# apple/ml-gmpi

Hardware: AMD Instinct MI355X
Metric: Mpix*planes/s (higher is better)
Workload: dtype f32; 1 GPU; FFHQ1024-shaped: 1024x1024, 96 planes, batch 4 views, bf16 storage; views_per_gpu=4, views_total=4, H=1024, W=1024, planes=96, variant=auto, strict_order=False, outputs=rgb+depth, parallelism=views sharded x1, poses=truncated-gaussian draw (seed 3) on every rank

## Files before the change

### include/gmpi_render.h

```cpp
#ifndef GMPI_RENDER_H
#define GMPI_RENDER_H

#include <stdint.h>

#ifdef __cplusplus
extern "C" {
#endif

#define GMPI_ABI_VERSION 2

enum { GMPI_DTYPE_F32 = 0, GMPI_DTYPE_BF16 = 1, GMPI_DTYPE_F16 = 2, GMPI_DTYPE_U8 = 3 };

enum {
    GMPI_FLAG_ALIGN_CORNERS = 1 << 0,
    GMPI_FLAG_OUT_PM1 = 1 << 1,
    GMPI_FLAG_CHECK_LAST_PLANE = 1 << 2,
    GMPI_FLAG_CHECK_RANGE = 1 << 3,
    GMPI_FLAG_STRICT_ORDER = 1 << 4,
    GMPI_FLAG_HINT_FRONTAL = 1 << 5,
    GMPI_FLAG_HINT_TILTED = 1 << 6,
    GMPI_FLAG_GRAD_OVERWRITE = 1 << 7,
    GMPI_FLAG_HINT_OBLIQUE = 1 << 8,
    GMPI_FLAG_ALL = (1 << 9) - 1
};

enum {
    GMPI_STATUS_OUT_OF_LAST_PLANE = 1u << 0,
    GMPI_STATUS_RGBA_RANGE = 1u << 1,
    GMPI_STATUS_CAMERA_BEHIND_PLANE = 1u << 2,
    GMPI_STATUS_BAD_VIEW_INDEX = 1u << 3
};
#define GMPI_STATUS_WORDS 4

enum {
    GMPI_VARIANT_AUTO = 0,
    GMPI_VARIANT_GATHER = 1,
    GMPI_VARIANT_LDS = 2,
    GMPI_VARIANT_WAVE = 3,
    GMPI_VARIANT_DMA = 4,
    GMPI_VARIANT_BAND = 5
};

enum {
    GMPI_OK = 0,
    GMPI_E_NULL = -1,
    GMPI_E_SHAPE = -2,
    GMPI_E_DTYPE = -3,
    GMPI_E_STRIDE = -4,
    GMPI_E_ABI = -5,
    GMPI_E_VARIANT = -6,
    GMPI_E_FLAGS = -7,
    GMPI_E_WORKSPACE = -8,
    GMPI_E_LAUNCH = -100
};

typedef struct GmpiRenderParams {
// ... 111 lines not shown
```

### ml-gmpi_amd/_lib.py

```python
import ctypes
import os
import subprocess

_PKG = os.path.dirname(os.path.abspath(__file__))
_SO = os.path.join(_PKG, "libgmpi_render.so")
_LIB = None

ABI_VERSION = 2
DTYPE_F32, DTYPE_BF16, DTYPE_F16 = 0, 1, 2
DTYPE_U8 = 3
FLAG_ALIGN_CORNERS, FLAG_OUT_PM1, FLAG_CHECK_LAST_PLANE, FLAG_CHECK_RANGE, FLAG_STRICT_ORDER, FLAG_HINT_FRONTAL, FLAG_HINT_TILTED = 1, 2, 4, 8, 16, 32, 64
FLAG_HINT_OBLIQUE = 256
FLAG_GRAD_OVERWRITE = 128
STATUS_OUT_OF_LAST_PLANE, STATUS_RGBA_RANGE, STATUS_CAMERA_BEHIND_PLANE, STATUS_BAD_VIEW_INDEX = 1, 2, 4, 8
STATUS_WORDS = 4
VARIANT_AUTO, VARIANT_GATHER, VARIANT_LDS, VARIANT_WAVE, VARIANT_DMA, VARIANT_BAND = 0, 1, 2, 3, 4, 5
VARIANTS = {"auto": VARIANT_AUTO, "gather": VARIANT_GATHER, "lds": VARIANT_LDS, "wave": VARIANT_WAVE, "band": VARIANT_BAND}

EXPORTS = (
    "gmpi_mpi_render_launch",
    "gmpi_render_workspace_bytes",
    "gmpi_render_backward_workspace_bytes",
    "gmpi_mpi_render_backward_launch",
    "gmpi_render_geometry_backward_workspace_bytes",
    "gmpi_mpi_render_geometry_backward_launch",
    "gmpi_mpi_render_backward_ex_launch",
    "gmpi_mpi_render_geometry_backward_ex_launch",
    "gmpi_mpi_render_shared_launch",
    "gmpi_mpi_render_shared_backward_launch",
    "gmpi_render_shared_supports",
    "gmpi_last_plane_uv_minmax_launch",
    "gmpi_rgba_range_check_launch",
    "gmpi_frames_to_uint8_launch",
    "gmpi_generate_rays_launch",
    "gmpi_alpha_depth_launch",
    "gmpi_light_blur_launch",
    "gmpi_light_shading_launch",
    "gmpi_light_apply_launch",
    "gmpi_light_apply_backward_launch",
    "gmpi_alpha_depth_backward_launch",
    "gmpi_alpha_depth_backward_ex_launch",
    "gmpi_selftest_division_launch",
    "gmpi_stream_probe_launch",
    "gmpi_query",
    "gmpi_version_string",
# ... 189 lines not shown
```

### ml-gmpi_amd/csrc/gmpi_abi.hip

```cpp
#include "gmpi_device.hpp"
#include "gmpi_shared.hpp"

#include "../../include/gmpi_render.h"

#include <atomic>
#include <cstdlib>

namespace gmpi {

hipError_t launch_gather(const KParams& p, int dtype, hipStream_t stream);
hipError_t launch_lds(const KParams& p, int dtype, int tune, hipStream_t stream);
hipError_t launch_backward(const KParams& p, int dtype, const float* g_rgb, const float* g_depth, const float* g_T, float* g_rgba,
                           const int64_t* gstride, bool tiles, hipStream_t stream);
bool lds_variant_supports(const KParams& p, int dtype);
int lds_variant_query(int what);
hipError_t launch_wave(const KParams& p, int dtype, int tune, hipStream_t stream);
bool wave_variant_supports(const KParams& p, int dtype);
hipError_t launch_band(const KParams& p, int dtype, int tune, hipStream_t stream);
bool band_variant_supports(const KParams& p, int dtype);
uint64_t band_workspace_bytes(const KParams& p, int dtype);
uint32_t* band_gate_words(const KParams& p, int dtype);
int band_pixels_wide(int dtype);
uint64_t backward_gather_workspace_bytes(const KParams& p);
uint64_t geometry_backward_workspace_bytes(const KParams& p, bool want_dhw);
hipError_t launch_shared(const KParams& p, int dtype, const SharedK& sh, hipStream_t stream);
hipError_t launch_shared_backward(const KParams& p, int dtype, const SharedK& sh, const SharedG& g, bool tiles, hipStream_t stream);
hipError_t launch_shared_forward(const KParams& p, int dtype, const SharedK& sh, hipStream_t stream);
bool shared_forward_supports(const KParams& p, int dtype, const SharedK& sh);
int shared_forward_query(int what);
hipError_t launch_u8(const KParams& p, hipStream_t stream);
bool u8_variant_supports(const KParams& p);
int u8_variant_query(int what);
hipError_t launch_backward_geometry(const KParams& p, int dtype, const float* g_rgb, const float* g_depth, const float* g_T, float* g_ray, float* g_eye,
                                    float* g_z, float* g_dhw, hipStream_t stream);

template <bool AC>
__global__ __launch_bounds__(256) void last_plane_uv_kernel(const KParams p, float* __restrict__ uv) {
    const int n = blockIdx.x;
    uint32_t bad_index = 0;
    const int m = view_mpi(p, n, bad_index);
    const float* dhw = p.dhw + (static_cast<int64_t>(m) * p.D + (p.D - 1)) * 3;
    const float d = dhw[0], ph = dhw[1], pw = dhw[2];
    const float ex = p.eye_pos[3 * n + 0], ey = p.eye_pos[3 * n + 1], ez = p.eye_pos[3 * n + 2];
    const float zdiff = d - ez;
    const int64_t HW = static_cast<int64_t>(p.H) * p.W;
    const float* rd = p.ray_dir + static_cast<int64_t>(n) * 3 * HW;
    const float inf = __builtin_inff();
    float mnu = inf, mxu = -inf, mnv = inf, mxv = -inf;
    bool nan = false;
    for (int64_t i = threadIdx.x; i < HW; i += blockDim.x) {
        float ix, iy, s, u, v;
        plane_coord<AC>(zdiff, ph, pw, ex, ey, rd[i], rd[HW + i], rd[2 * HW + i], 1.0f, 1.0f, ix, iy, s, u, v);
        nan |= (u != u) || (v != v);
        mnu = fminf(mnu, u), mxu = fmaxf(mxu, u), mnv = fminf(mnv, v), mxv = fmaxf(mxv, v);
    }
// ... 550 lines not shown
int gmpi_selftest_division_launch(uint64_t pairs, uint32_t seed, uint64_t* mismatches, void* stream) {
    if (mismatches == nullptr) return GMPI_E_NULL;
    if (pairs == 0) return GMPI_OK;
    const uint64_t want = (pairs + 255) / 256;
    const unsigned blocks = static_cast<unsigned>(want < 256u * 64u ? want : 256u * 64u);
    hipLaunchKernelGGL(selftest_division_kernel, dim3(blocks), dim3(256), 0, static_cast<hipStream_t>(stream), pairs, seed,
                       reinterpret_cast<unsigned long long*>(mismatches));
    return hip_rc(hipGetLastError());
}

int gmpi_stream_probe_launch(const void* buf, uint64_t bytes, uint32_t* sink, void* stream) {
    if (buf == nullptr) return GMPI_E_NULL;
    if (reinterpret_cast<uintptr_t>(buf) % 4 != 0) return GMPI_E_STRIDE;
    if (bytes < 4) return GMPI_OK;
    hipLaunchKernelGGL(stream_probe_kernel, dim3(256 * 2), dim3(256), 0, static_cast<hipStream_t>(stream), static_cast<const uint32_t*>(buf),
                       static_cast<int64_t>(bytes / 4), sink);
    return hip_rc(hipGetLastError());
}

int gmpi_query(int32_t what) {
    switch (what) {
        case 0: return GMPI_ABI_VERSION;
        case 1: return static_cast<int>(sizeof(GmpiRenderParams));
        case 2: return 950;
        case 3: case 4: case 5: return lds_variant_query(what);
        case 6: return 1;
        case 7: return 0;
        case 8: return 1;
        case 9: return static_cast<int>(kAutoBandMin);
        case 10: return static_cast<int>(kAutoBandMinF32);
        case 11: return 1;
        case 12: case 13: case 14: return shared_forward_query(what);
        case 16: case 17: case 18: case 20: return u8_variant_query(what);
        default: return -1;
    }
}

const char* gmpi_version_string(void) { return "ml-gmpi_amd 0.3 (gfx950, ABI 2)"; }

}
```

### ml-gmpi_amd/csrc/render_band.hip

```cpp
#include "gmpi_device.hpp"

#include <algorithm>
#include <cstdlib>
#include <type_traits>


namespace gmpi {
namespace band {

constexpr int kNT = 1024;
constexpr int SBW = 64, SBH = 8;
constexpr float kBoxEps = 1.0f / 64;
constexpr int kWindowCols16 = 2, kWindowCols32 = 2, kWindowCols32Deep = 2, kDeepPlanes = 128;
constexpr int kViewRotation = 1;
constexpr int kRunPieces = 2;
constexpr int kTicketTail = 16;
constexpr float kCoordLimit = 16384.0f;

typedef uint32_t u32x4 __attribute__((ext_vector_type(4)));
template <int V> using ic = std::integral_constant<int, V>;

template <int D0, int STEP>
__device__ __forceinline__ void dma16x2(uint32_t voff, uint32_t soff1, const u32x4& rsrc, uint32_t lds_dst, uint64_t m0, uint64_t m1);

#ifndef GMPI_BAND_PPT16
#define GMPI_BAND_PPT16 2
#endif
#ifndef GMPI_BAND_PPT32
#define GMPI_BAND_PPT32 2
#endif
template <typename TexT> struct Geo {
    static constexpr int kES = static_cast<int>(sizeof(TexT));
    static constexpr int NSB = kES == 2 ? 4 : 2;
    static constexpr int PPT = kES == 2 ? GMPI_BAND_PPT16 : GMPI_BAND_PPT32;
    static constexpr int WPS = SBH / PPT;
    static constexpr int kSubLanes = 64 * WPS;
    static constexpr int kThreads = NSB * kSubLanes;
    static constexpr int kWavesPerSimd = kThreads / 128;
    static_assert(kThreads <= kNT && SBH % PPT == 0, "waves");
    static constexpr int kTPI = 16 / kES;
    static constexpr int kCols = kES == 2 ? 10 : 20;
    static constexpr int kLineBytes = kCols * 16;
    static constexpr int kRowBytes = 4 * kLineBytes;
    static constexpr int kIPR = 4 * kCols;
    static constexpr int kMaxRows = 15;
    static constexpr int kCapItems = kMaxRows * kIPR;
    static constexpr int kSubBytes = kCapItems * 16;
    static constexpr int kBufBytes = NSB * kSubBytes;
    static constexpr int kRPP = kSubLanes / kIPR;
    static constexpr int kPassItems = kRPP * kIPR;
    static constexpr int kNP = (kMaxRows + kRPP - 1) / kRPP;
    static_assert(kNP == 3 || kNP == 5, "passes");
    static constexpr int kOffBytes = kThreads * 4;
    static constexpr int kLdsBytes = kOffBytes + 2 * kBufBytes;
};
static_assert(Geo<bf16_t>::kLdsBytes * 2 <= 160 * 1024 && Geo<f16_t>::kLdsBytes * 2 <= 160 * 1024 && Geo<float>::kLdsBytes * 2 <= 160 * 1024, "2 workgroups per CU");

__device__ __forceinline__ void dma16(uint32_t voff, uint32_t soff, const u32x4& rsrc, uint32_t lds_dst, uint64_t mask) {
    uint64_t save;
    asm volatile("s_mov_b64 %0, exec\n\ts_mov_b64 exec, %4\n\ts_mov_b32 m0, %3\n\ts_nop 0\n\tbuffer_load_dwordx4 %1, %2, %5 offen lds\n\ts_mov_b64 exec, %0"
                 : "=&s"(save) : "v"(voff), "s"(rsrc), "s"(lds_dst), "s"(mask), "s"(soff) : "memory");
}
template <int D0, int STEP>
__device__ __forceinline__ void dma16x3(uint32_t voff, uint32_t soff1, uint32_t soff2, const u32x4& rsrc, uint32_t lds_dst, uint64_t m0, uint64_t m1, uint64_t m2) {
    uint64_t save;
    asm volatile("s_mov_b64 %0, exec\n\t"
                 "s_mov_b64 exec, %4\n\ts_add_i32 m0, %3, %9\n\ts_nop 0\n\tbuffer_load_dwordx4 %1, %2, 0 offen lds\n\t"
                 "s_mov_b64 exec, %5\n\ts_add_i32 m0, %3, %10\n\ts_nop 0\n\tbuffer_load_dwordx4 %1, %2, %7 offen lds\n\t"
                 "s_mov_b64 exec, %6\n\ts_add_i32 m0, %3, %11\n\ts_nop 0\n\tbuffer_load_dwordx4 %1, %2, %8 offen lds\n\t"
                 "s_mov_b64 exec, %0"
                 : "=&s"(save) : "v"(voff), "s"(rsrc), "s"(lds_dst), "s"(m0), "s"(m1), "s"(m2), "s"(soff1), "s"(soff2), "i"(D0), "i"(D0 + STEP), "i"(D0 + 2 * STEP)
                 : "memory", "scc");
}
template <int D0, int STEP>
__device__ __forceinline__ void dma16x2(uint32_t voff, uint32_t soff1, const u32x4& rsrc, uint32_t lds_dst, uint64_t m0, uint64_t m1) {
    uint64_t save;
    asm volatile("s_mov_b64 %0, exec\n\t"
                 "s_mov_b64 exec, %4\n\ts_add_i32 m0, %3, %7\n\ts_nop 0\n\tbuffer_load_dwordx4 %1, %2, 0 offen lds\n\t"
                 "s_mov_b64 exec, %5\n\ts_add_i32 m0, %3, %8\n\ts_nop 0\n\tbuffer_load_dwordx4 %1, %2, %6 offen lds\n\t"
                 "s_mov_b64 exec, %0"
                 : "=&s"(save) : "v"(voff), "s"(rsrc), "s"(lds_dst), "s"(m0), "s"(m1), "s"(soff1), "i"(D0), "i"(D0 + STEP)
                 : "memory", "scc");
}
template <int D0, int STEP>
__device__ __forceinline__ void dma16x4(uint32_t voff, uint32_t s1, uint32_t s2, uint32_t s3, const u32x4& rsrc, uint32_t lds_dst, uint64_t m0, uint64_t m1, uint64_t m2, uint64_t m3) {
    uint64_t save;
    asm volatile("s_mov_b64 %0, exec\n\t"
                 "s_mov_b64 exec, %4\n\ts_add_i32 m0, %3, %11\n\ts_nop 0\n\tbuffer_load_dwordx4 %1, %2, 0 offen lds\n\t"
                 "s_mov_b64 exec, %5\n\ts_add_i32 m0, %3, %12\n\ts_nop 0\n\tbuffer_load_dwordx4 %1, %2, %8 offen lds\n\t"
// ... 178 lines not shown
            }
            __syncthreads();
            band_id = __builtin_amdgcn_readfirstlane(*word);
            __syncthreads();
        }
    }
#ifdef GMPI_TUNE
    if (p.flags & (1u << 19)) band_id = static_cast<int>(blockIdx.x % 8) * ((n_bands + 7) / 8) + static_cast<int>(blockIdx.x / 8);
#endif
    if (band_id >= n_bands) return;
    int n, brem;
    item_to_view(p, band_id, bands_x * bands_y, n, brem);
    if (view_gated_out(p, n)) return;
    int bxi, byi;
    band_pos(brem, bands_x, bands_y, p.band_cols, bxi, byi);
#ifdef GMPI_TUNE
    const bool stamp = (p.flags & (1u << 22)) != 0 && p.status != nullptr;
    uint64_t stamp_start = 0;
    if (stamp) asm volatile("s_memrealtime %0\n\ts_waitcnt lgkmcnt(0)" : "=s"(stamp_start));
#endif

    const int tid = threadIdx.x;
    auto fresh_tid = [&]() { int t = tid; asm volatile("" : "+v"(t)); return t; };
    const int wave = __builtin_amdgcn_readfirstlane(tid >> 6);
    const int sb = wave / WPS, wj = wave % WPS;
    const int lane = tid & 63;
    uint32_t bad_w = 0;
    View vw = view_setup<AC>(p, n, bad_w);
    vw.cx = cx, vw.cy = cy;
    const int D = p.D, H = p.H, W = p.W;
    const float* __restrict__ dhw = vw.dhw;
    const float ex = vw.ex, ey = vw.ey, ez = vw.ez;
    constexpr bool check_range = CHECK;
    const int64_t HW = vw.HW;
    const float* __restrict__ rdv = vw.rays;
    const TexT* __restrict__ vol = static_cast<const TexT*>(p.rgba) + static_cast<int64_t>(vw.m) * p.s_mpi;
    const int64_t s_chan = p.s_chan, s_row = p.s_row;

    check_camera_behind(p, vw, brem == 0 && tid == 0);

    const int px = bxi * (NSB * SBW) + sb * SBW + lane;
    const int py0 = byi * SBH + wj;
    const int pxc = min(px, W - 1);
    float rx[PPT], ry[PPT], rz[PPT], rcp_rz[PPT];
    Accum A[PPT];
#pragma unroll
    for (int q = 0; q < PPT; ++q) {
        const int64_t pix = static_cast<int64_t>(min(py0 + WPS * q, H - 1)) * W + pxc;
        rx[q] = rdv[pix], ry[q] = rdv[HW + pix], rz[q] = rdv[2 * HW + pix];
        rcp_rz[q] = 1.0f / rz[q];
    }
    auto ray_dot = [&](int q) { return gmpi::ray_dot(vw, rx[q], ry[q], rz[q]); };

    auto loader_pos = [&](int& l_col, int& l_line, int& l_row, bool& l_on) {
        const int t = fresh_tid() & (kSubLanes - 1);
        l_line = t / kCols, l_col = t - l_line * kCols, l_row = l_line >> 2, l_on = t < kPassItems;
    };
    {
        int l_col, l_line, l_row;
        bool l_on;
        loader_pos(l_col, l_line, l_row, l_on);
        reinterpret_cast<uint32_t*>(smem + 2 * kBufBytes)[tid] = static_cast<uint32_t>(l_row * s_row + (l_line & 3) * s_chan + kTPI * l_col) * static_cast<uint32_t>(kES);
    }
    const uint32_t pass_off = static_cast<uint32_t>(kRPP * s_row) * static_cast<uint32_t>(kES), pass_off2 = 2 * pass_off;
    const uint32_t pass_off3 = 3 * pass_off, pass_off4 = 4 * pass_off;
    const uint32_t sub_base = tile_base + static_cast<uint32_t>(sb * kSubBytes);
    const uint32_t wave_dst = sub_base + static_cast<uint32_t>(wj) * 1024u;

#ifdef GMPI_TUNE
    const bool abl_noload = (p.flags & (1u << 16)) != 0, abl_nocomp = (p.flags & (1u << 17)) != 0, abl_noissue = (p.flags & (1u << 18)) != 0;
    const bool abl_nobar = (p.flags & (1u << 20)) != 0, abl_norec = (p.flags & (1u << 21)) != 0;
#else
    constexpr bool abl_noload = false, abl_nocomp = false, abl_noissue = false, abl_nobar = false, abl_norec = false;
#endif

#ifdef GMPI_PROF
    uint32_t prof_acc[8] = {0, 0, 0, 0, 0, 0, 0, 0};
    uint64_t prof_last, prof_start;
    asm volatile("s_memtime %0\n\ts_waitcnt lgkmcnt(0)" : "=s"(prof_start));
    prof_last = prof_start;
#define GMPI_STAMP(i) do { uint64_t now_; asm volatile("s_memtime %0\n\ts_waitcnt lgkmcnt(0)" : "=s"(now_)); prof_acc[i] += static_cast<uint32_t>(now_ - prof_last); prof_last = now_; } while (0)
#else
#define GMPI_STAMP(i) do { } while (0)
#endif

    const uint4* __restrict__ myrec = recs + (static_cast<int64_t>(band_id) * D * NSB + sb);
    const uint4* __restrict__ mypl = pl + static_cast<int64_t>(n) * D * kPlU4;
    constexpr int kRecStep = NSB;

    if (hdr[band_id] != 0) {
#pragma unroll
        for (int q = 0; q < PPT; ++q) {
            const float dot = ray_dot(q);
            for (int t = 0; t < D; ++t) {
                uint32_t gbad = 0;
                gather_plane<TexT, AC, STRICT>(p, vw, vol, t, dhw[3 * t] - ez, dhw[3 * t + 1], dhw[3 * t + 2], rx[q], ry[q], rz[q], dot, std::bool_constant<CHECK>{}, gbad, A[q]);
                if (check_range && __any(gbad != 0)) bad_w |= GMPI_STATUS_RGBA_RANGE;
            }
        }
    } else {
        float dots[PPT];
#pragma unroll
        for (int q = 0; q < PPT; ++q) dots[q] = STRICT ? ray_dot(q) : 0.0f;
        uint64_t m_cur[kNP];
        int dims_cur = 0;
        bool three = false;
        int np_cur = kNP - 1;
#pragma unroll
        for (int r = 0; r < kNP; ++r) m_cur[r] = 0;

        auto issue = [&](const uint4& rl, uint32_t g_off, auto ub) {
            constexpr int U = decltype(ub)::value;
            const int dims = static_cast<int>(rl.z);
            const u32x4 rsrc = {static_cast<uint32_t>(__builtin_amdgcn_readfirstlane(static_cast<int>(rl.x))),
                                static_cast<uint32_t>(__builtin_amdgcn_readfirstlane(static_cast<int>(rl.y))), 0x80000000u, 0x00020000u};
            if (dims >= 0) {
                if (dims != dims_cur) {
                    const int nq = dims & 31, rows = dims >> 5;
                    dims_cur = dims;
                    three = rows > (kNP - 1) * kRPP;
                    np_cur = max((rows + kRPP - 1) / kRPP, 3);
                    int l_col, l_line, l_row;
                    bool l_on;
                    loader_pos(l_col, l_line, l_row, l_on);
#pragma unroll
                    for (int r = 0; r < kNP; ++r) {
                        m_cur[r] = __ballot(l_on && l_col < nq && l_row + r * kRPP < rows);
                        if (abl_noload) m_cur[r] = 0;
                    }
                }
// ... 104 lines not shown
        };
        auto taps32_land = [&](auto nb, u32x2_t (&v)[4]) {
            constexpr int N = decltype(nb)::value;
            asm volatile("s_waitcnt lgkmcnt(%4)" : "+v"(v[0]), "+v"(v[1]), "+v"(v[2]), "+v"(v[3]) : "i"(N));
        };
        auto pixel = [&](int q, const float4& rf, const float2& rg) {
            Coords c;
            coords(q, rf, rg, c);
            Footprint f;
            f.nw = c.nw, f.ne = c.ne, f.sw = c.sw, f.se = c.se;
            uint32_t t[8];
            float smp[4];
            taps(ic<0>{}, c.a_tap, t);
            if (check_range) tap_fold8(t);
            smp[0] = bilerp<STRICT>(tapf(t[0]), tapf(t[1]), tapf(t[2]), tapf(t[3]), f);
            smp[1] = bilerp<STRICT>(tapf(t[4]), tapf(t[5]), tapf(t[6]), tapf(t[7]), f);
            taps(ic<1>{}, c.a_tap, t);
            if (check_range) tap_fold8(t);
            smp[2] = bilerp<STRICT>(tapf(t[0]), tapf(t[1]), tapf(t[2]), tapf(t[3]), f);
            smp[3] = bilerp<STRICT>(tapf(t[4]), tapf(t[5]), tapf(t[6]), tapf(t[7]), f);
            blend<STRICT>(A[q], smp[0], smp[1], smp[2], smp[3], c.s, dots[q]);
        };


        uint4 Ln, Fc;
        uint32_t rhh_c, gp_c;
        uint32_t g_off = 0;
#ifdef GMPI_PROF
        constexpr bool piped = false, pipedG = false;
#else
        constexpr bool piped = BF && !STRICT && PPT == 2 && kNP == 3;
        constexpr bool pipedG = !STRICT && !piped;
#endif
        auto stage = [&](int tt, auto ub) {
            constexpr int U = decltype(ub)::value;
            if (!abl_nobar) wg_barrier();
            GMPI_STAMP(0);
            if (tt + 1 < D && !abl_noissue) issue(Ln, g_off, ic<1 - U>{});
            GMPI_STAMP(3);
            const float4 rf = make_float4(__uint_as_float(Fc.x), __uint_as_float(Fc.y), __uint_as_float(Fc.z), __uint_as_float(Fc.w));
            const float2 rg = make_float2(__uint_as_float(rhh_c), static_cast<float>(static_cast<int>(gp_c) + static_cast<int>(tile_base) + U * kBufBytes));
            if constexpr (piped) {
                if (!abl_nocomp) {
                    uint32_t ta[8], tb[8];
                    Coords p0, p1;
                    Footprint f;
                    float smp[4];
                    coords(0, rf, rg, p0);
                    taps_issue(ic<0>{}, p0.a_tap, ta);
                    taps_issue(ic<1>{}, p0.a_tap, tb);
                    coords(1, rf, rg, p1);
                    asm volatile("" : "+v"(p1.s), "+v"(p1.nw), "+v"(p1.ne), "+v"(p1.sw), "+v"(p1.se), "+v"(p1.a_tap));
                    taps_land(ic<8>{}, ta);
                    if (check_range) tap_fold8(ta);
                    f.nw = p0.nw, f.ne = p0.ne, f.sw = p0.sw, f.se = p0.se;
                    smp[0] = bilerp<false>(tapf(ta[0]), tapf(ta[1]), tapf(ta[2]), tapf(ta[3]), f);
                    smp[1] = bilerp<false>(tapf(ta[4]), tapf(ta[5]), tapf(ta[6]), tapf(ta[7]), f);
                    asm volatile("" : "+v"(smp[0]), "+v"(smp[1]));
                    taps_issue(ic<0>{}, p1.a_tap, ta);
                    taps_land(ic<8>{}, tb);
                    if (check_range) tap_fold8(tb);
                    smp[2] = bilerp<false>(tapf(tb[0]), tapf(tb[1]), tapf(tb[2]), tapf(tb[3]), f);
                    smp[3] = bilerp<false>(tapf(tb[4]), tapf(tb[5]), tapf(tb[6]), tapf(tb[7]), f);
                    blend<false>(A[0], smp[0], smp[1], smp[2], smp[3], p0.s, dots[0]);
                    asm volatile("" : "+v"(A[0].T), "+v"(A[0].r), "+v"(A[0].g), "+v"(A[0].b), "+v"(A[0].z));
                    taps_issue(ic<1>{}, p1.a_tap, tb);
                    taps_land(ic<8>{}, ta);
                    if (check_range) tap_fold8(ta);
                    f.nw = p1.nw, f.ne = p1.ne, f.sw = p1.sw, f.se = p1.se;
// ... 66 lines not shown
                            issueB(pn);
                            pc = pn;
                        }
                    };
                    coords(0, rf, rg, pc);
                    issueA(pc);
                    issueB(pc);
                    px_step(ic<0>{});
                    if constexpr (PPT > 1) px_step(ic<1>{});
                    if constexpr (PPT > 2) px_step(ic<2>{});
                    if constexpr (PPT > 3) px_step(ic<3>{});
                    static_assert(PPT <= 4, "pixel slots");
                }
            } else {
                GMPI_STAMP(2);
                if (!abl_nocomp) {
#pragma unroll
                    for (int q = 0; q < PPT; ++q) {
                        pixel(q, rf, rg);
                        GMPI_STAMP(5 + q);
                    }
                }
            }
            if (!abl_norec) {
                gp_c = Ln.w;
                Ln = myrec[static_cast<int64_t>(tt + 2) * kRecStep];
                Fc = mypl[(tt + 1) * kPlU4], rhh_c = mypl[(tt + 1) * kPlU4 + 1].x;
            }
            static_assert(PPT <= 4 && kNP <= 5, "pixel slots / check passes");
        };
#pragma unroll
        for (int q = 0; q < PPT; ++q)
            asm volatile("" : "+v"(rx[q]), "+v"(ry[q]), "+v"(rz[q]), "+v"(rcp_rz[q]), "+v"(A[q].T), "+v"(A[q].r), "+v"(A[q].g), "+v"(A[q].b), "+v"(A[q].z));
        __syncthreads();
        g_off = reinterpret_cast<const uint32_t*>(smem + 2 * kBufBytes)[fresh_tid()];
        issue(myrec[0], g_off, ic<0>{});
        Fc = mypl[0], rhh_c = mypl[1].x, gp_c = myrec[0].w, Ln = myrec[kRecStep];
        for (int t = 0; t < D; t += 2) {
            stage(t, ic<0>{});
            if (t + 1 < D) stage(t + 1, ic<1>{});
        }
        if (check_range) {
            constexpr uint32_t kOne = F16 ? 0x3c00u : BF ? 0x3f80u : 0x3f800000u, kNegZero = BF ? 0x8000u : 0x80000000u;
            const uint32_t mx = BF ? chk_acc >> 16 : chk_acc;
#ifdef GMPI_TUNE
            if (p.status != nullptr && mx > kOne) { atomicMax(p.status + 1, mx); atomicMax(p.status + 2, static_cast<uint32_t>(band_id)); atomicMax(p.status + 3, static_cast<uint32_t>(tid)); }
#endif
            if (__any(mx > kOne)) {
                if (__any(mx > kOne && mx != kNegZero)) bad_w |= GMPI_STATUS_RGBA_RANGE;
                else {
                    int l_col, l_line, l_row;
                    bool l_on;
                    loader_pos(l_col, l_line, l_row, l_on);
                    const uint32_t g0 = reinterpret_cast<const uint32_t*>(smem + 2 * kBufBytes)[fresh_tid()];
                    bool lane_bad = false;
                    for (int t = 0; t < D; ++t) {
                        const uint4 rl = myrec[static_cast<int64_t>(t) * kRecStep];
                        const Shape h = shape_unpack(rl.z);
                        const int nq = h.nq;
                        const uint32_t clo = h.clo, ncol = h.ncol, llo = 4 * h.rlo, nline = 4 * h.nrow;
                        const unsigned char* org = reinterpret_cast<const unsigned char*>((static_cast<uint64_t>(rl.y) << 32) | rl.x);
                        for (int r = 0; r < kNP; ++r) {
                            const bool in = l_on && l_col < nq && (static_cast<uint32_t>(l_col) - clo < ncol) && (static_cast<uint32_t>(l_line + 4 * r * kRPP) - llo < nline);
                            if (!in) continue;
                            const uint4 q = *reinterpret_cast<const uint4*>(org + g0 + static_cast<uint32_t>(r) * pass_off);
                            const uint32_t d[4] = {q.x, q.y, q.z, q.w};
#pragma unroll
                            for (int c = 0; c < 4; ++c) {
                                if (BF) lane_bad |= !((d[c] & 0xffffu) <= kOne || (d[c] & 0xffffu) == kNegZero) || !((d[c] >> 16) <= kOne || (d[c] >> 16) == kNegZero);
                                else lane_bad |= !(d[c] <= kOne || d[c] == kNegZero);
                            }
                        }
                    }
                    if (__any(lane_bad)) bad_w |= GMPI_STATUS_RGBA_RANGE;
                }
            }
        }
    }

    uint32_t bad = bad_w;
    const LastPlane lp = last_plane(p, vw);
    const int px_e = bxi * (NSB * SBW) + sb * SBW + (fresh_tid() & 63);
#pragma unroll
    for (int q = 0; q < PPT; ++q) {
        const int py = byi * SBH + wj + WPS * q;
        if (leaves_last_plane<AC>(vw, lp, rx[q], ry[q], rz[q])) bad |= GMPI_STATUS_OUT_OF_LAST_PLANE;
        store_pixel<STRICT>(p, n, HW, static_cast<int64_t>(py) * W + px_e, A[q], ray_dot(q), px_e < W && py < H);
    }
    report_status(p.status, bad);
// ... 28 lines not shown
    band_grid(p, nsb, bx, by, nb);
    return ws_hdr_bytes(nb, p.N) + ws_pl_bytes(p) + (static_cast<uint64_t>(nb) * p.D + 2) * nsb * 16;
}

template <typename TexT>
static hipError_t launch_t(const KParams& p, hipStream_t stream) {
    constexpr int NSB = Geo<TexT>::NSB;
    int bands_x, bands_y, n_bands;
    band_grid(p, NSB, bands_x, bands_y, n_bands);
    const int group_items = bands_x * bands_y * (p.view_to_mpi == nullptr ? p.views_per_mpi : 1);
    const int tail = std::min(p.band_tail, (group_items + 7) / 8);
    const dim3 grid(xcd_grid_per_group(group_items, n_bands) + 8u * static_cast<unsigned>(tail)), block(Geo<TexT>::kThreads);
    uint32_t* tickets = static_cast<uint32_t*>(p.ws) + n_bands + p.N;
    const bool acf = p.flags & GMPI_FLAG_ALIGN_CORNERS;
    const float cx = acf ? static_cast<float>(p.Wt - 1) * 0.5f : static_cast<float>(p.Wt), cy = acf ? static_cast<float>(p.Ht - 1) * 0.5f : static_cast<float>(p.Ht);
    uint32_t* hdr = static_cast<uint32_t*>(p.ws);
    uint4* pl = reinterpret_cast<uint4*>(static_cast<unsigned char*>(p.ws) + ws_hdr_bytes(n_bands, p.N));
    uint4* recs = reinterpret_cast<uint4*>(static_cast<unsigned char*>(p.ws) + ws_hdr_bytes(n_bands, p.N) + ws_pl_bytes(p));
    const dim3 tgrid(static_cast<unsigned>(n_bands)), tblock(static_cast<unsigned>(std::min(1024, (p.D * NSB + 63) / 64 * 64)));
    dispatch_bool(acf, [&](auto AC) {
        hipLaunchKernelGGL((band_table_kernel<TexT, decltype(AC)::value>), tgrid, tblock, 0, stream, p, bands_x, bands_y, n_bands, cx, cy, recs, pl, hdr, tickets);
    });
    dispatch_ac_strict(p.flags, [&](auto AC, auto STRICT) {
        dispatch_bool(p.flags & GMPI_FLAG_CHECK_RANGE, [&](auto CHECK) {
            hipLaunchKernelGGL((render_band_kernel<TexT, decltype(AC)::value, decltype(STRICT)::value, decltype(CHECK)::value>), grid, block, 0, stream, p, bands_x,
                               bands_y, n_bands, cx, cy, recs, pl, hdr, tickets);
        });
    });
    return hipGetLastError();
}

}

uint64_t band_workspace_bytes(const KParams& p, int dtype) { return band::ws_bytes(p, band::nsb_of(dtype)); }
int band_pixels_wide(int dtype) { return band::nsb_of(dtype) * band::SBW; }

uint32_t* band_gate_words(const KParams& p, int dtype) {
    int bx, by, nb;
    band::band_grid(p, band::nsb_of(dtype), bx, by, nb);
    return static_cast<uint32_t*>(p.ws) + nb;
}

bool band_variant_supports(const KParams& p, int dtype) {
    if (dtype < 0 || dtype > 2) return false;
    const int nsb = band::nsb_of(dtype), bw = nsb * band::SBW;
    if (p.ws == nullptr || p.ws_bytes < band::ws_bytes(p, nsb) || reinterpret_cast<uintptr_t>(p.ws) % 256 != 0) return false;
    if (static_cast<int64_t>(p.N) * p.D * ((p.W + bw - 1) / bw) * ((p.H + 7) / 8) > (int64_t(1) << 28)) return false;
    const int es = dtype == 0 ? 4 : 2;
    if (!volume_stages_in_items(p, dtype)) return false;
    if (p.Ht > 8192 || p.Wt > 8192) return false;
    const int64_t span = 3 * p.s_chan + 18 * p.s_row + 128;
    if (span >= (int64_t(1) << 31) / es) return false;
    return true;
}

hipError_t launch_band(const KParams& p0, int dtype, int tune, hipStream_t stream) {
    KParams p = p0;
    p.band_cols = dtype != 0 ? band::kWindowCols16 : p.D > band::kDeepPlanes ? band::kWindowCols32Deep : band::kWindowCols32;
    p.band_rot = band::kViewRotation, p.band_split = band::kRunPieces, p.band_tail = band::kTicketTail;
#ifdef GMPI_TUNE
    p.flags |= static_cast<uint32_t>((tune >> 8) & 127) << 16;
    static const int env_order = [] { const char* e = getenv("GMPI_TUNE_ORDER"); return e ? atoi(e) : 0; }();
    if (env_order > 0) p.band_cols = env_order;
    static const int env_rot = [] { const char* e = getenv("GMPI_TUNE_ROT"); return e ? atoi(e) : -1; }();
    if (env_rot >= 0) p.band_rot = env_rot;
    static const int env_split = [] { const char* e = getenv("GMPI_TUNE_SPLIT"); return e ? atoi(e) : 0; }();
// ... 12 lines not shown
```

### ml-gmpi_amd/hip_mpi.py

```python
import atexit
import collections
import contextlib
import ctypes
import sys
import threading
import warnings
import weakref
from typing import List, Optional, Sequence, Union

import numpy as np
import torch
from torch import nn

from . import _lib
from .quantized import is_interleaved

_DTYPES = {torch.float32: _lib.DTYPE_F32, torch.bfloat16: _lib.DTYPE_BF16, torch.float16: _lib.DTYPE_F16, torch.uint8: _lib.DTYPE_U8}


def _refuse_uint8(what: str, *tensors) -> None:
    for t in tensors:
        if t is not None and t.dtype is torch.uint8:
            raise TypeError(f"{what} does not take uint8 storage: pass dequantize_volume(q) (ml_gmpi_amd.quantized), or render the RGBA volume "
                            "with MPI.render_views / MPIRenderer.render, which read the 8-bit codes as they are")
# ... 303 lines not shown
    return t.to(dev, torch.float32).contiguous()


def _view_index(views_per_mpi, view_to_mpi, M: int, N: int, dev: torch.device):
    uniform = 0
    if view_to_mpi is None:
        if isinstance(views_per_mpi, int):
            uniform = views_per_mpi
        elif len(set(views_per_mpi)) == 1 and len(views_per_mpi) == M:
            uniform = int(views_per_mpi[0])
        else:
            assert len(views_per_mpi) == M and sum(views_per_mpi) == N
            view_to_mpi = torch.repeat_interleave(torch.arange(M, dtype=torch.int32),
                                                  torch.tensor(list(views_per_mpi))).to(dev)
        if uniform:
            assert N == M * uniform, f"{N} views for {M} MPIs x {uniform}"
    if view_to_mpi is not None:
        view_to_mpi = view_to_mpi.to(dev, torch.int32).contiguous()
        assert view_to_mpi.shape == (N,)
    return uniform, view_to_mpi


def _cat(parts: Union[torch.Tensor, Sequence[torch.Tensor]]) -> torch.Tensor:
    if isinstance(parts, torch.Tensor):
        return parts
    return parts[0] if len(parts) == 1 else torch.cat(list(parts), dim=0)


class MPI(nn.Module):

    DEFAULT_RANGE_CHECK = "touched"

    def __init__(self, align_corners=True, variant: str = "auto", strict_order: bool = False,
                 range_check: Optional[str] = None, on_out_of_plane: str = "exit", backward: str = "atomic", geometry_grad: bool = False):
        super().__init__()
        self.geometry_grad = bool(geometry_grad)
        self._align_corners = align_corners
        if range_check is None:
            range_check = type(self).DEFAULT_RANGE_CHECK
        assert variant in _lib.VARIANTS, variant
        assert range_check in ("touched", "full", "off"), range_check
        assert on_out_of_plane in ("exit", "raise"), on_out_of_plane
        assert backward in ("atomic", "gather"), backward
        self.backward = backward
        self.variant = variant
        self.strict_order = strict_order
        self.range_check = range_check
        self.on_out_of_plane = on_out_of_plane
        self._full_check_passed = None
        self.shared_lds_fallbacks = 0

    def __getstate__(self):
        state = self.__dict__.copy()
        state["_full_check_passed"] = None
        return state

    @staticmethod
    def _volume_fingerprint(rgba: torch.Tensor):
        anchor = rgba._base if rgba._base is not None else rgba
        return anchor, (rgba.data_ptr(), tuple(rgba.shape), tuple(rgba.stride()), rgba.dtype, rgba._version, str(rgba.device))

    def _full_check_needed(self, rgba: torch.Tensor) -> bool:
        hit = self._full_check_passed
        if hit is None:
            return True
        anchor, fp = self._volume_fingerprint(rgba)
        return not (hit[0]() is anchor and hit[1] == fp)

# ... 124 lines not shown
                        p.variant = _lib.VARIANT_AUTO
                        self.shared_lds_fallbacks += 1
                        _warn_lds_fallback()
                _call("gmpi_mpi_render_shared_launch", dev, ctypes.byref(p), ctypes.byref(sc), stream=stream)
            else:
                _call("gmpi_mpi_render_launch", dev, ctypes.byref(p), stream=stream)
            res = dict(color=color, depth=depth, T=T, status=status)
            if _in_autograd_fn:
                res["_bwd"] = (p, keep) if _shared is None else (p, keep, (sh_rgb, sh_bg))
            if ring is not None:
                ring.host_words[slot].copy_(status, non_blocking=True)
                ev = torch.cuda.Event()
                ev.record(current)
                ring.pending.append((slot, ev, self, p, keep, c2w_mat, sphere_c))
            elif not defer_status:
                self._settle(status, p, keep, c2w_mat, sphere_c, rgba_in if _shared is None and checked else None)
            return res

    def _autograd_bridge(self, rgba, dhw, ray_dir, eye_pos, z_dir, shared):
        geometry = self.geometry_grad and any(t.requires_grad for t in (dhw, ray_dir, eye_pos, z_dir))
        if shared is None:
            return (_RenderFunction, (rgba,)) if rgba.requires_grad or geometry else None
        if geometry:
            raise NotImplementedError("the shared-colour render has no gradient w.r.t. the plane geometry or the camera tensors "
                                      "(geometry_grad=True): render the expanded volume (expand_shared_color) with render_views for that")
        if rgba.requires_grad or any(t is not None and t.requires_grad for t in shared):
            return _SharedRenderFunction, (shared[0], rgba, shared[1])
        return None

    def _flags(self, out_pm1, check_last_plane, frontal_hint, tilted_hint, oblique_hint) -> int:
        return ((_lib.FLAG_ALIGN_CORNERS if self._align_corners else 0) | (_lib.FLAG_OUT_PM1 if out_pm1 else 0)
                | (_lib.FLAG_CHECK_LAST_PLANE if check_last_plane else 0) | (_lib.FLAG_CHECK_RANGE if self.range_check != "off" else 0)
                | (_lib.FLAG_STRICT_ORDER if self.strict_order else 0) | (_lib.FLAG_HINT_FRONTAL if frontal_hint else 0)
                | (_lib.FLAG_HINT_TILTED if tilted_hint else 0) | (_lib.FLAG_HINT_OBLIQUE if oblique_hint else 0))

    def _settle(self, status, p, keep, c2w_mat, sphere_c, fully_checked) -> None:
        try:
            self.raise_on_status(status, params=p, keep=keep, c2w_mat=c2w_mat, sphere_c=sphere_c)
        except BaseException:
            if status.is_cuda:
                status.zero_()
            self._full_check_passed = None
            raise
        if fully_checked is not None:
            self._full_check_record(fully_checked)

    def render_views_shared(self, rgb: torch.Tensor, alpha: torch.Tensor, dhw: torch.Tensor, ray_dir: torch.Tensor, eye_pos: torch.Tensor,
                            z_dir: torch.Tensor, background: Optional[torch.Tensor] = None, variant: Optional[str] = None, **kwargs):
        from .shared_color import _check
        _check(rgb, alpha, background)
        assert "_shared" not in kwargs
        return self.render_views(alpha, dhw, ray_dir, eye_pos, z_dir, _shared=(rgb, background), _shared_variant=variant, **kwargs)

    def raise_on_status(self, status: torch.Tensor, params=None, keep=None, c2w_mat=None, sphere_c=None):
        word = int(status[0].item())
        if word == 0:
            return
        if status.is_cuda:
            status.zero_()
        if word & _lib.STATUS_BAD_VIEW_INDEX:
            raise IndexError("view_to_mpi holds an index outside [0, #mpi)")
        if word & _lib.STATUS_RGBA_RANGE:
            raise AssertionError("Expected alpha to be within the the range [0, 1]")
        if word & _lib.STATUS_CAMERA_BEHIND_PLANE:
            dist = keep[1][..., 0].flatten().tolist() if keep is not None else "?"
            eye0 = keep[3][0].tolist() if keep is not None else "?"
            raise AssertionError(f"Camera must be placed closer to origin than MPI. {dist}, {eye0}")
# ... 156 lines not shown
```

### ml-gmpi_amd/renderer.py

```python
import logging

import numpy as np
import torch

from .hip_mpi import MPI, _call, _cat
from .pinhole import gen_cam
from .plane_geometry import compute_plane_dhws, sample_distance
from .poses import draw_angle_noise, gen_sphere_path, gen_sphere_paths_ahead, host_math

logger = logging.getLogger("ml_gmpi_amd")

EPS = 1e-6
_COS_FRONTAL = 0.98006658
_COS_TILTED = 0.86280707
_COS_OBLIQUE = 0.93937271

PRESETS = {
    "FFHQ": dict(plane_min_d=0.95, plane_max_d=1.12, cam_fov=12.6, sphere_center_z=1.0, sphere_r=1.0,
                 horizontal_mean=0.0, horizontal_std=0.289, vertical_mean=0.0, vertical_std=0.127,
                 cam_pose_n_truncated_stds=2),
    "MetFaces": dict(plane_min_d=0.95, plane_max_d=1.12, cam_fov=12.6, sphere_center_z=1.0, sphere_r=1.0,
                     horizontal_mean=0.0, horizontal_std=0.339, vertical_mean=0.0, vertical_std=0.133,
                     cam_pose_n_truncated_stds=2),
    "AFHQCat": dict(plane_min_d=2.55, plane_max_d=2.8, cam_fov=13.39, sphere_center_z=2.7, sphere_r=2.7,
                    horizontal_mean=0.0, horizontal_std=0.19, vertical_mean=0.0, vertical_std=0.15,
                    cam_pose_n_truncated_stds=3),
}


def make_renderer(preset="FFHQ", n_planes=96, device=None, align_corners=True, confined=True, **over):
    kw = dict(PRESETS[preset])
    kw.update(n_mpi_planes=n_planes, plan_spatial_enlarge_factor=1.001, plane_distances_sample_method="inverse",
              cam_sample_method="truncated_gaussian", mpi_align_corners=align_corners, use_confined_volume=confined,
              device=device if device is not None else torch.device("cuda"))
    kw.update(over)
    return MPIRenderer(**kw)


class MPIRenderer:
    def __init__(self, *, n_mpi_planes, plane_min_d, plane_max_d, plan_spatial_enlarge_factor,
                 plane_distances_sample_method, cam_fov, sphere_center_z, sphere_r, horizontal_mean, horizontal_std,
                 vertical_mean, vertical_std, cam_pose_n_truncated_stds, cam_sample_method, mpi_align_corners=True,
                 use_xyz_ztype="depth", use_normalized_xyz=False, normalized_xyz_range="-11",
                 use_confined_volume=False, device=torch.device("cpu"),
                 kernel_variant="auto", strict_order=False, range_check=None, on_out_of_plane="exit",
                 ray_backend="auto", status_mode="sync", backward="atomic", geometry_grad=False):
        self.mpi = MPI(align_corners=mpi_align_corners, variant=kernel_variant, strict_order=strict_order,
                       range_check=range_check, on_out_of_plane=on_out_of_plane, backward=backward, geometry_grad=geometry_grad)
        self.use_confined_volume = use_confined_volume
        self.n_mpi_planes = n_mpi_planes
        self.plane_min_d = plane_min_d
        self.plane_max_d = plane_max_d
        self.plan_spatial_enlarge_factor = plan_spatial_enlarge_factor
        self.plane_distances_sample_method = plane_distances_sample_method
        self.mpi_tex_h = None
        self.mpi_tex_w = None
        self.cam_fov = cam_fov
        self.sphere_center = np.array([0, 0, sphere_center_z])
        self.sphere_r = sphere_r
        self.horizontal_mean = horizontal_mean
        self.horizontal_std = horizontal_std
        self.vertical_mean = vertical_mean
        self.vertical_std = vertical_std
        self.cam_pose_n_truncated_stds = cam_pose_n_truncated_stds
        self.cam_sample_method = cam_sample_method
        self.device = device
        assert ray_backend in ("auto", "torch", "hip"), ray_backend
        if ray_backend == "auto":
            ray_backend = "hip" if torch.device(device).type == "cuda" else "torch"
        self.ray_backend = ray_backend
        assert status_mode in ("lag", "sync"), status_mode
        self.status_mode = "lag" if status_mode == "lag" else False
        self._batched_cam = None
        self._dhw_dev = None
        self._dhw_rep = None
        self._spec = None
        self._det_poses = {}
        self._ray_bufs = {}
        self._frontal = False
        self._tilted = False
        self._oblique = False
# ... 350 lines not shown
```

Before: 522,200 Mpix*planes/s.

## Add workgroup-voted early ray termination to band renderer when transmittance falls below cutoff

Adds early exit to the band compositing kernel. Every few planes each wave votes in LDS on whether any pixel still has transmittance above 2^-30, and the workgroup stops processing planes once none does. The gather path gets a per-wave break on the same test. This saves the remaining plane loads and blending for opaque pixels. The cost is an extra barrier and vote per group of planes, a small LDS addition, and output that is no longer bit-exact, since contributions below the cutoff are dropped.

```diff
diff --git a/include/gmpi_render.h b/include/gmpi_render.h
--- a/include/gmpi_render.h
+++ b/include/gmpi_render.h
@@ -21,7 +21,8 @@
     GMPI_FLAG_HINT_TILTED = 1 << 6,
     GMPI_FLAG_GRAD_OVERWRITE = 1 << 7,
     GMPI_FLAG_HINT_OBLIQUE = 1 << 8,
-    GMPI_FLAG_ALL = (1 << 9) - 1
+    GMPI_FLAG_NO_EARLY_EXIT = 1 << 10,
+    GMPI_FLAG_ALL = ((1 << 9) - 1) | (1 << 10)
 };
 
 enum {
diff --git a/ml-gmpi_amd/_lib.py b/ml-gmpi_amd/_lib.py
--- a/ml-gmpi_amd/_lib.py
+++ b/ml-gmpi_amd/_lib.py
@@ -11,6 +11,7 @@
 DTYPE_U8 = 3
 FLAG_ALIGN_CORNERS, FLAG_OUT_PM1, FLAG_CHECK_LAST_PLANE, FLAG_CHECK_RANGE, FLAG_STRICT_ORDER, FLAG_HINT_FRONTAL, FLAG_HINT_TILTED = 1, 2, 4, 8, 16, 32, 64
 FLAG_HINT_OBLIQUE = 256
+FLAG_NO_EARLY_EXIT = 1024
 FLAG_GRAD_OVERWRITE = 128
 STATUS_OUT_OF_LAST_PLANE, STATUS_RGBA_RANGE, STATUS_CAMERA_BEHIND_PLANE, STATUS_BAD_VIEW_INDEX = 1, 2, 4, 8
 STATUS_WORDS = 4
diff --git a/ml-gmpi_amd/csrc/gmpi_abi.hip b/ml-gmpi_amd/csrc/gmpi_abi.hip
--- a/ml-gmpi_amd/csrc/gmpi_abi.hip
+++ b/ml-gmpi_amd/csrc/gmpi_abi.hip
@@ -21,6 +21,8 @@
 uint64_t band_workspace_bytes(const KParams& p, int dtype);
 uint32_t* band_gate_words(const KParams& p, int dtype);
 int band_pixels_wide(int dtype);
+uint32_t band_early_exit_cut_bits();
+int band_early_exit_vote_planes();
 uint64_t backward_gather_workspace_bytes(const KParams& p);
 uint64_t geometry_backward_workspace_bytes(const KParams& p, bool want_dhw);
 hipError_t launch_shared(const KParams& p, int dtype, const SharedK& sh, hipStream_t stream);
@@ -637,6 +639,8 @@
         case 11: return 1;
         case 12: case 13: case 14: return shared_forward_query(what);
         case 16: case 17: case 18: case 20: return u8_variant_query(what);
+        case 22: return static_cast<int>(band_early_exit_cut_bits());
+        case 23: return band_early_exit_vote_planes();
         default: return -1;
     }
 }
diff --git a/ml-gmpi_amd/csrc/render_band.hip b/ml-gmpi_amd/csrc/render_band.hip
--- a/ml-gmpi_amd/csrc/render_band.hip
+++ b/ml-gmpi_amd/csrc/render_band.hip
@@ -15,6 +15,13 @@
 constexpr int kViewRotation = 1;
 constexpr int kRunPieces = 2;
 constexpr int kTicketTail = 16;
+constexpr float kTCut = 0x1p-30f;
+constexpr uint32_t kTCutBits = 0x30800000u;
+#ifndef GMPI_BAND_VOTE
+#define GMPI_BAND_VOTE 8
+#endif
+constexpr int kVote = GMPI_BAND_VOTE;
+static_assert(kVote % 2 == 0 && kVote >= 2, "a vote lands on a buffer-pair boundary");
 constexpr float kCoordLimit = 16384.0f;
 
 typedef uint32_t u32x4 __attribute__((ext_vector_type(4)));
@@ -52,9 +59,11 @@
     static constexpr int kNP = (kMaxRows + kRPP - 1) / kRPP;
     static_assert(kNP == 3 || kNP == 5, "passes");
     static constexpr int kOffBytes = kThreads * 4;
-    static constexpr int kLdsBytes = kOffBytes + 2 * kBufBytes;
+    static constexpr int kVoteOff = 2 * kBufBytes + kOffBytes;
+    static constexpr int kLdsBytes = kVoteOff + 8;
 };
-static_assert(Geo<bf16_t>::kLdsBytes * 2 <= 160 * 1024 && Geo<f16_t>::kLdsBytes * 2 <= 160 * 1024 && Geo<float>::kLdsBytes * 2 <= 160 * 1024, "2 workgroups per CU");
+constexpr int lds_granules(int bytes) { return (bytes + 1279) / 1280 * 1280; }
+static_assert(lds_granules(Geo<bf16_t>::kLdsBytes) * 2 <= 160 * 1024 && lds_granules(Geo<f16_t>::kLdsBytes) * 2 <= 160 * 1024 && lds_granules(Geo<float>::kLdsBytes) * 2 <= 160 * 1024, "2 workgroups per CU");
 
 __device__ __forceinline__ void dma16(uint32_t voff, uint32_t soff, const u32x4& rsrc, uint32_t lds_dst, uint64_t mask) {
     uint64_t save;
@@ -299,6 +308,7 @@
     const float* __restrict__ dhw = vw.dhw;
     const float ex = vw.ex, ey = vw.ey, ez = vw.ez;
     constexpr bool check_range = CHECK;
+    const bool early_exit = !STRICT && p.T_out == nullptr && (p.flags & GMPI_FLAG_NO_EARLY_EXIT) == 0;
     const int64_t HW = vw.HW;
     const float* __restrict__ rdv = vw.rays;
     const TexT* __restrict__ vol = static_cast<const TexT*>(p.rgba) + static_cast<int64_t>(vw.m) * p.s_mpi;
@@ -363,6 +373,7 @@
                 uint32_t gbad = 0;
                 gather_plane<TexT, AC, STRICT>(p, vw, vol, t, dhw[3 * t] - ez, dhw[3 * t + 1], dhw[3 * t + 2], rx[q], ry[q], rz[q], dot, std::bool_constant<CHECK>{}, gbad, A[q]);
                 if (check_range && __any(gbad != 0)) bad_w |= GMPI_STATUS_RGBA_RANGE;
+                if (early_exit && !__any(__float_as_uint(A[q].T) >= kTCutBits)) break;
             }
         }
     } else {
@@ -533,9 +544,18 @@
         constexpr bool piped = BF && !STRICT && PPT == 2 && kNP == 3;
         constexpr bool pipedG = !STRICT && !piped;
 #endif
-        auto stage = [&](int tt, auto ub) {
+        typedef __attribute__((address_space(3))) volatile uint32_t lds_word;
+        lds_word* vote = reinterpret_cast<lds_word*>((lds_byte*)smem + G::kVoteOff);
+        auto verdict = [&](int tt) -> bool {
+            const int w = (tt / kVote - 1) & 1;
+            vote[w ^ 1] = 0u;
+            const uint32_t alive = vote[w];
+            return __builtin_amdgcn_readfirstlane(static_cast<int>(alive)) == 0;
+        };
+        auto stage = [&](int tt, auto ub, auto nb) {
             constexpr int U = decltype(ub)::value;
-            if (!abl_nobar) wg_barrier();
+            if constexpr (decltype(nb)::value == 0)
+                if (!abl_nobar) wg_barrier();
             GMPI_STAMP(0);
             if (tt + 1 < D && !abl_noissue) issue(Ln, g_off, ic<1 - U>{});
             GMPI_STAMP(3);
@@ -668,13 +688,32 @@
 #pragma unroll
         for (int q = 0; q < PPT; ++q)
             asm volatile("" : "+v"(rx[q]), "+v"(ry[q]), "+v"(rz[q]), "+v"(rcp_rz[q]), "+v"(A[q].T), "+v"(A[q].r), "+v"(A[q].g), "+v"(A[q].b), "+v"(A[q].z));
+        if (fresh_tid() < 2) vote[fresh_tid()] = 0u;
         __syncthreads();
         g_off = reinterpret_cast<const uint32_t*>(smem + 2 * kBufBytes)[fresh_tid()];
         issue(myrec[0], g_off, ic<0>{});
         Fc = mypl[0], rhh_c = mypl[1].x, gp_c = myrec[0].w, Ln = myrec[kRecStep];
-        for (int t = 0; t < D; t += 2) {
-            stage(t, ic<0>{});
-            if (t + 1 < D) stage(t + 1, ic<1>{});
+        int d_done = D;
+        const int vstep = !STRICT && early_exit ? kVote : 0x40000000;
+        for (int t0 = 0; t0 < D; t0 += vstep) {
+            if (!abl_nobar) wg_barrier();
+            if constexpr (!STRICT)
+                if (t0 != 0 && verdict(t0)) { d_done = t0; break; }
+            stage(t0, ic<0>{}, ic<1>{});
+            if (t0 + 1 < D) stage(t0 + 1, ic<1>{}, ic<0>{});
+            const int t1 = min(t0 + vstep, D);
+            for (int t = t0 + 2; t < t1; t += 2) {
+                stage(t, ic<0>{}, ic<0>{});
+                if (t + 1 < D) stage(t + 1, ic<1>{}, ic<0>{});
+            }
+            if constexpr (!STRICT) {
+                if (t0 + vstep < D) {
+                    uint32_t tmax = __float_as_uint(A[0].T);
+#pragma unroll
+                    for (int q = 1; q < PPT; ++q) tmax = max(tmax, __float_as_uint(A[q].T));
+                    if (__any(tmax >= kTCutBits) && (fresh_tid() & 63) == 0) vote[((t0 + vstep) / kVote - 1) & 1] = 1u;
+                }
+            }
         }
         if (check_range) {
             constexpr uint32_t kOne = F16 ? 0x3c00u : BF ? 0x3f80u : 0x3f800000u, kNegZero = BF ? 0x8000u : 0x80000000u;
@@ -690,7 +729,7 @@
                     loader_pos(l_col, l_line, l_row, l_on);
                     const uint32_t g0 = reinterpret_cast<const uint32_t*>(smem + 2 * kBufBytes)[fresh_tid()];
                     bool lane_bad = false;
-                    for (int t = 0; t < D; ++t) {
+                    for (int t = 0; t < d_done; ++t) {
                         const uint4 rl = myrec[static_cast<int64_t>(t) * kRecStep];
                         const Shape h = shape_unpack(rl.z);
                         const int nq = h.nq;
@@ -785,6 +824,9 @@
 
 }
 
+uint32_t band_early_exit_cut_bits() { return band::kTCutBits; }
+int band_early_exit_vote_planes() { return band::kVote; }
+static_assert(__builtin_bit_cast(uint32_t, band::kTCut) == band::kTCutBits, "the cut and its pattern");
 uint64_t band_workspace_bytes(const KParams& p, int dtype) { return band::ws_bytes(p, band::nsb_of(dtype)); }
 int band_pixels_wide(int dtype) { return band::nsb_of(dtype) * band::SBW; }
 
diff --git a/ml-gmpi_amd/hip_mpi.py b/ml-gmpi_amd/hip_mpi.py
--- a/ml-gmpi_amd/hip_mpi.py
+++ b/ml-gmpi_amd/hip_mpi.py
@@ -359,8 +359,10 @@
     DEFAULT_RANGE_CHECK = "touched"
 
     def __init__(self, align_corners=True, variant: str = "auto", strict_order: bool = False,
-                 range_check: Optional[str] = None, on_out_of_plane: str = "exit", backward: str = "atomic", geometry_grad: bool = False):
+                 range_check: Optional[str] = None, on_out_of_plane: str = "exit", backward: str = "atomic", geometry_grad: bool = False,
+                 early_exit: bool = True):
         super().__init__()
+        self.early_exit = bool(early_exit)
         self.geometry_grad = bool(geometry_grad)
         self._align_corners = align_corners
         if range_check is None:
@@ -551,7 +553,8 @@
         return ((_lib.FLAG_ALIGN_CORNERS if self._align_corners else 0) | (_lib.FLAG_OUT_PM1 if out_pm1 else 0)
                 | (_lib.FLAG_CHECK_LAST_PLANE if check_last_plane else 0) | (_lib.FLAG_CHECK_RANGE if self.range_check != "off" else 0)
                 | (_lib.FLAG_STRICT_ORDER if self.strict_order else 0) | (_lib.FLAG_HINT_FRONTAL if frontal_hint else 0)
-                | (_lib.FLAG_HINT_TILTED if tilted_hint else 0) | (_lib.FLAG_HINT_OBLIQUE if oblique_hint else 0))
+                | (_lib.FLAG_HINT_TILTED if tilted_hint else 0) | (_lib.FLAG_HINT_OBLIQUE if oblique_hint else 0)
+                | (0 if getattr(self, "early_exit", True) else _lib.FLAG_NO_EARLY_EXIT))
 
     def _settle(self, status, p, keep, c2w_mat, sphere_c, fully_checked) -> None:
         try:
diff --git a/ml-gmpi_amd/renderer.py b/ml-gmpi_amd/renderer.py
--- a/ml-gmpi_amd/renderer.py
+++ b/ml-gmpi_amd/renderer.py
@@ -44,9 +44,10 @@
                  use_xyz_ztype="depth", use_normalized_xyz=False, normalized_xyz_range="-11",
                  use_confined_volume=False, device=torch.device("cpu"),
                  kernel_variant="auto", strict_order=False, range_check=None, on_out_of_plane="exit",
-                 ray_backend="auto", status_mode="sync", backward="atomic", geometry_grad=False):
+                 ray_backend="auto", status_mode="sync", backward="atomic", geometry_grad=False, early_exit=True):
         self.mpi = MPI(align_corners=mpi_align_corners, variant=kernel_variant, strict_order=strict_order,
-                       range_check=range_check, on_out_of_plane=on_out_of_plane, backward=backward, geometry_grad=geometry_grad)
+                       range_check=range_check, on_out_of_plane=on_out_of_plane, backward=backward, geometry_grad=geometry_grad,
+                       early_exit=early_exit)
         self.use_confined_volume = use_confined_volume
         self.n_mpi_planes = n_mpi_planes
         self.plane_min_d = plane_min_d
```

Result: faster. 938,200 Mpix*planes/s, median of 6 (+79.7%).
